# xp3i4/linear

Hardware: AMD Instinct MI355X
Metric: reads/sec (whole node) + HBM GB/s on seed lookup, 10 kb reads vs GRCh38 (higher is better)
Workload: dtype u64

## Files before the change

linear_amd/csrc/lnr_hd.h:

```cpp
#pragma once
#include <stdint.h>
#include <limits.h>
#include "ref_sort.h"

namespace lnr {

typedef uint64_t u64;
typedef int64_t i64;
typedef uint32_t u32;
typedef int32_t i32;
typedef uint16_t u16;
typedef uint8_t u8;

struct UP { u64 first, second; };

static const u64 ANCHOR_ZERO = 1ULL << 20;
static const u64 F_END = 1ULL << 60, F_STRAND = 1ULL << 61, F_RECD = 1ULL << 62, F_MAIN = 1ULL << 63;
static const u64 VALUE_MASK_DSTR = ((1ULL << 60) - 1) | F_STRAND;
static const u64 MAX_CORD_ID = (1ULL << 10) - 1, MAX_CORD_X = (1ULL << 30) - 1;

LNR_HD inline u64 cord_x(u64 v) { return (v >> 20) & ((1ULL << 30) - 1); }
LNR_HD inline u64 cord_y(u64 v) { return v & 0xfffffULL; }
LNR_HD inline u64 cord_strand(u64 v) { return (v >> 61) & 1ULL; }
LNR_HD inline u64 cord_id(u64 v) { return (v >> 50) & 1023ULL; }
LNR_HD inline u64 cord_x40(u64 v) { return (v >> 20) & 0xffffffffffULL; }
LNR_HD inline u64 mk_cord(u64 idx, u64 y, u64 s) { return (idx << 20) + y + (s << 61); }
LNR_HD inline u64 create_cord(u64 id, u64 x, u64 y, u64 s) { return mk_cord((id << 30) + x, y, s); }
LNR_HD inline u64 shift_cord(u64 v, i64 x, i64 y) { return x < 0 ? v - ((u64)(-x) << 20) + (u64)y : v + ((u64)x << 20) + (u64)y; }
LNR_HD inline bool is_end(u64 v) { return (v & F_END) != 0; }
LNR_HD inline u64 hit2cord(u64 a) { return ((a + ((a & 0xfffffULL) << 20) - (ANCHOR_ZERO << 20)) & VALUE_MASK_DSTR) & ~(1ULL << 62); }
LNR_HD inline u64 anchor_x(u64 a) { return cord_x(hit2cord(a)); }
LNR_HD inline i64 labs64(i64 v) { return v < 0 ? -v : v; }
LNR_HD inline i64 max64(i64 a, i64 b) { return a > b ? a : b; }
LNR_HD inline i64 min64(i64 a, i64 b) { return a < b ? a : b; }
LNR_HD inline u64 umin64(u64 a, u64 b) { return a < b ? a : b; }
LNR_HD inline u64 umax64(u64 a, u64 b) { return a > b ? a : b; }
LNR_HD inline int consecutive(u64 c1, u64 c2, u64 thd) {
    u64 x1 = cord_x(c1), x2 = cord_x(c2), y1 = cord_y(c1), y2 = cord_y(c2);
    return !cord_strand(c1 ^ c2) && x1 <= x2 && y1 <= y2 && x2 - x1 < thd && y2 - y1 < thd;
}
LNR_HD inline UP forward_y(UP se, u64 L) {
    UP r;
    if (cord_strand(se.first)) { r.first = L - cord_y(se.second) - 1; r.second = L - cord_y(se.first) - 1; }
    else { r.first = cord_y(se.first); r.second = cord_y(se.second); }
    return r;
}

LNR_HD inline bool lnr_is_leader() {
#if defined(__HIP_DEVICE_COMPILE__)
    return (threadIdx.x & 63) == 0;
#else
    return true;
#endif
}
LNR_HD inline void lnr_wave_sync() {
#if defined(__HIP_DEVICE_COMPILE__)
    __builtin_amdgcn_fence(__ATOMIC_RELEASE, "workgroup");
    __builtin_amdgcn_wave_barrier();
    __builtin_amdgcn_fence(__ATOMIC_ACQUIRE, "workgroup");
#endif
}
LNR_HD inline u32 lnr_uni32(u32 v) {
#if defined(__HIP_DEVICE_COMPILE__)
    return (u32)__builtin_amdgcn_readfirstlane((int)v);
#else
    return v;
#endif
}
LNR_HD inline u64 lnr_uni64(u64 v) { return ((u64)lnr_uni32((u32)(v >> 32)) << 32) | (u64)lnr_uni32((u32)v); }
template <class T>
struct Vec {
    T *p; u32 n, cap; int *ovf;
    LNR_HD void init(T *p_, u32 cap_, int *ovf_) { p = p_; n = 0; cap = cap_; ovf = ovf_; }
    LNR_HD void push(const T &v) { if (n < cap) p[n++] = v; else *ovf = 1; }
    LNR_HD void push_u(const T &v) {
        if (n < cap) { if (lnr_is_leader()) p[n] = v; n++; }
        else if (lnr_is_leader()) *ovf = 1;
    }
    LNR_HD T &operator[](u32 i) { return p[i]; }
    LNR_HD T &back() { return p[n - 1]; }
};
struct Arena {
    char *base; u64 off, cap; int ovf; Arena *next;
    LNR_HD void init(void *b, u64 c) { base = (char *)b; off = 0; cap = c; ovf = 0; next = nullptr; }
    template <class T> LNR_HD T *get(u64 n) {
        u64 bytes = (n * sizeof(T) + 15) & ~15ULL;
        Arena *a = this;
        while (a->off + bytes > a->cap) {
            if (!a->next) { a->ovf = 1; ovf = 1; return (T *)base; }
            a = a->next;
        }
        T *r = (T *)(a->base + a->off);
        a->off += bytes;
        return r;
    }
};
LNR_HD inline u64 job_scratch_bytes(u64 cap) { return (cap + 2) * 160 + 1024; }
LNR_HD inline u64 tail_scratch_bytes(u64 cap) { return cap * 240 + 8192; }

LNR_HD inline int lnr_popc64(u64 v) {
#if defined(__HIP_DEVICE_COMPILE__)
    return __popcll(v);
#else
    return __builtin_popcountll(v);
#endif
}
struct PackedSeq {
    const u64 *pk; const u32 *nm; u64 L;
    LNR_HD u8 operator[](u64 i) const {
        u64 j = i < L ? i : L;
        u32 n = nm[j >> 5]; u64 w = pk[j >> 5];
        u32 v = (u32)(w >> (2 * (j & 31))) & 3;
        return (u8)(((n >> (j & 31)) & 1) ? 4 : v);
    }
    LNR_HD int sum20(u64 p) const {
        u64 w = p >> 5; u32 sh = (u32)(p & 31);
        u64 lo = pk[w], hi = pk[w + 1];
        u64 bits = sh ? (lo >> (2 * sh)) | (hi << (64 - 2 * sh)) : lo;
        bits &= (1ULL << 40) - 1;
        u64 nb = ((((u64)nm[w + 1] << 32) | nm[w]) >> sh) & ((1ULL << 20) - 1);
        return lnr_popc64(bits & 0x5555555555555555ULL) + 2 * lnr_popc64(bits & 0xAAAAAAAAAAAAAAAAULL) + 4 * lnr_popc64(nb);
    }
};
struct ByteSeq {
    const u8 *p; u64 L;
    LNR_HD u8 operator[](u64 i) const { if (i >= L) return 0; u8 b = p[i]; return b > 4 ? (u8)4 : b; }
};
struct SeedOut { u32 X; u32 Y; u32 strand; };

template <int SPAN, class Seq> LNR_HD inline int shape_init_skip_t(const Seq &s) {
    u64 k = 0, count = 0;
    while (count < (u64)SPAN) {
        if (s[k + count] == 4) { k += count + 1; count = 0; }
        else count++;
    }
    return (int)k;
}
template <class Seq> LNR_HD inline int shape_init_skip(const Seq &s) { return shape_init_skip_t<21>(s); }
template <int SPAN, class Seq> LNR_HD inline int shape_const_t(const Seq &s, u64 init_at, int ks, u64 k0) {
    int a = 0, b = 0;
    for (int i = 0; i < SPAN - 1; i++) { a += s[init_at + ks + i]; b += s[k0 + i]; }
    return -3 * SPAN + 2 * a - 2 * b;
}
template <class Seq> LNR_HD inline int shape_const(const Seq &s, u64 init_at, int ks, u64 k0) { return shape_const_t<21>(s, init_at, ks, k0); }
LNR_HD inline int shape_const(const PackedSeq &s, u64 init_at, int ks, u64 k0) {
    return -63 + 2 * s.sum20(init_at + (u64)ks) - 2 * s.sum20(k0);
}
template <int SPAN, int WEIGHT, class Seq> LNR_HD inline SeedOut seed_sample_t(const Seq &s, u64 k, u64 k0, u64 init_at, int ks, int C) {
    u64 h = 0, crh = 0;
    int W = 0;
    u64 n = k - k0 + 1;
    int stale = n < (u64)SPAN ? (int)(SPAN - n) : 0;
    for (int p = 0; p < SPAN; p++) {
        u64 real = s[k + p];
        W += (int)real;
        u64 v = p < stale ? (u64)s[init_at + ks + n - 1 + p] : real;
        h = (h << 2) + v;
        crh |= ((3 - v) & 3) << (2 * p);
    }
    int x = C + 2 * W;
    u64 v2 = x > 0 ? (h & ((1ULL << (2 * SPAN)) - 1)) : crh;
    u64 X = (1ULL << (2 * SPAN)) - 1, t = 0;
    for (unsigned kk = 64 - 2 * SPAN; kk <= 64 - 2 * WEIGHT; kk += 2) {
        u64 v1 = v2 << kk >> (64 - 2 * WEIGHT);
        if (X > v1) { X = v1; t = kk; }
    }
    u64 Y = 0;
    if (x > 0) {
        i64 d = (i64)(t >> 1) + SPAN + WEIGHT - 32;
        for (i64 i = d; i < d + 4; i++) { u64 val = s[(u64)((i64)k + i)]; Y = val > 3 ? (Y << 2) : (Y << 2) + val; }
    } else {
        i64 d = 31 - WEIGHT - (i64)(t >> 1);
        for (i64 i = d; i > d - 4; i--) { i64 val = 3 - (i64)s[(u64)((i64)k + i)]; Y = val < 0 ? (Y << 2) : (Y << 2) + (u64)val; }
    }
    SeedOut o; o.X = (u32)X; o.Y = (u32)Y; o.strand = x > 0 ? 0 : 1;
    return o;
}
template <class Seq> LNR_HD inline SeedOut seed_sample(const Seq &s, u64 k, u64 k0, u64 init_at, int ks, int C) { return seed_sample_t<21, 13>(s, k, k0, init_at, ks, C); }
LNR_HD inline u64 lnr_brev64(u64 v) {
#if defined(__HIP_DEVICE_COMPILE__)
    return __brevll(v);
#else
    v = ((v >> 1) & 0x5555555555555555ULL) | ((v & 0x5555555555555555ULL) << 1);
    v = ((v >> 2) & 0x3333333333333333ULL) | ((v & 0x3333333333333333ULL) << 2);
    v = ((v >> 4) & 0x0F0F0F0F0F0F0F0FULL) | ((v & 0x0F0F0F0F0F0F0F0FULL) << 4);
    v = ((v >> 8) & 0x00FF00FF00FF00FFULL) | ((v & 0x00FF00FF00FF00FFULL) << 8);
    v = ((v >> 16) & 0x0000FFFF0000FFFFULL) | ((v & 0x0000FFFF0000FFFFULL) << 16);
    return (v >> 32) | (v << 32);
#endif
}
LNR_HD inline bool seed_sample_packed(const u64 *pk, const u32 *nm, u64 k, u64 k0, int C, SeedOut &o) {
    if (k - k0 + 1 < 21 || k < 4) return false;
    u64 s0 = k - 4;
    u64 w = s0 >> 5;
    u32 sh = (u32)(s0 & 31);
    u64 nbits = (((u64)nm[w + 1] << 32) | nm[w]) >> sh;
    if (nbits & ((1ULL << 29) - 1)) return false;
    u64 lo = pk[w], hi = pk[w + 1];
    u64 span = sh ? (lo >> (2 * sh)) | (hi << (64 - 2 * sh)) : lo;
    const u64 M42 = (1ULL << 42) - 1;
    u64 win = (span >> 8) & M42;
    int W = lnr_popc64(win & 0x5555555555555555ULL) + 2 * lnr_popc64(win & 0xAAAAAAAAAAAAAAAAULL);
    int x = C + 2 * W;
    u64 v2;
    if (x > 0) {
        u64 r = lnr_brev64(win) >> 22;
        v2 = ((r & 0x2AAAAAAAAAAULL) >> 1) | ((r & 0x15555555555ULL) << 1);
    } else v2 = (~win) & M42;
    u32 v2lo = (u32)v2, v2hi = (u32)(v2 >> 32);
    u32 best = 0xffffffffu;
#pragma unroll
    for (u32 i = 0; i < 9; i++) {
        u32 p = 16 - 2 * i;
        u32 f = p ? ((v2lo >> p) | (v2hi << (32 - p))) : v2lo;
        u32 key = ((f & 0x3ffffffu) << 4) | i;
        best = key < best ? key : best;
    }
    u64 X = best >> 4, t = 22 + 2 * (best & 15u);
    u32 Y;
    if (x > 0) {
        u32 q = (u32)(t >> 1) + 2 + 4;
        u32 b = (u32)(span >> (2 * q)) & 0xFF;
// ... 502 lines not shown
    i32 dx = (i32)((u32)(c11 >> 20) & 0x3fffffffu) - (i32)((u32)(c22 >> 20) & 0x3fffffffu);
    if (dx < 0 || dy < 0 || cord_strand(c11 ^ c22) || dx > 20000 || dy > 20000) return INT_MIN;
    u32 ux = (u32)dx, uy = (u32)dy;
    u32 da = ux > uy ? ux - uy : uy - ux;
    u32 D = uy > 100u ? uy : 100u; D = D > ux ? D : ux;
#if defined(__HIP_DEVICE_COMPILE__)
    float inv = __builtin_amdgcn_rcpf((float)D);
#else
    float inv = 1.0f / (float)D;
#endif
    u32 n = 100u * da;
    u32 q = (u32)((float)n * inv);
    i32 r = (i32)(n - q * D);
    q = r < 0 ? q - 1 : ((u32)r >= D ? q + 1 : q);
    if (da > 100u || q > 50u) {
        if (ux < uy) return (int)(100 - 30) - (int)(uy / 1000u) - (int)(ux / 100u);
        return (int)(100 - 30) - (int)(uy / 100u) - (int)(ux / 1000u);
    }
    return 100 - (int)(uy / 95u);
}
LNR_HD inline int block_score3(u64 c11, u64 c12, u64 c21, u64 c22, u64 L, int strand) {
    i64 dx, dy;
    if (cord_strand(c11) != (u64)strand) {
        if (cord_strand(c22) != (u64)strand) { dy = (i64)(cord_y(c21) - cord_y(c12)); dx = (i64)(cord_x(c21) - cord_x(c12)); }
        else { dy = (i64)(L - cord_y(c12) - 1 - cord_y(c22)); dx = (i64)(cord_x(c11) - cord_x(c22)); }
    } else {
        if (cord_strand(c22) != (u64)strand) { dy = (i64)(cord_y(c11) - L + 1 + cord_y(c21)); dx = (i64)(cord_x(c11) - cord_x(c22)); }
        else { dy = (i64)(cord_y(c11) - cord_y(c22)); dx = (i64)(cord_x(c11) - cord_x(c22)); }
    }
    int f_type = (int)cord_strand(c11 ^ c22);
    i64 thd_min_dx = -(i64)L;
    i64 thd_max_dy = (i64)((float)L * 1.0f);
    i64 dx_ = labs64(dx), dy_ = labs64(dy), da = dx - dy;
    int score = 0;
    if (dy < -80 || dy > thd_max_dy || dx < thd_min_dx || dx_ > 15000) score = INT_MIN;
    else {
        i64 sdy = dy_ > 2000 ? min64(dy_ / 25 - 50, 70) : dy_ / 40;
        i64 sdx = dx_ > 2000 ? min64(dx_ / 25 - 50, 70) : dx_ / 40;
        if (f_type == 1) { if (dx > thd_min_dx) score = (int)(75 - sdy); }
        else if (da < -max64(dx_ / 4, 50)) { if (dx > -50) score = (int)(80 - sdx); else score = (int)(80 - sdy); }
        else if (da > max64(dy / 4, 50)) score = (int)(80 - sdy);
        else score = (int)(100 - sdy);
    }
    return score;
}
LNR_HD inline void best_chains2(const u64 *hits, const UP *sep, const i32 *sep_score, u32 nb, Rec r, u64 L, int which, int strand) {
    for (u32 i = 0; i < nb; i++) {
        int j_str = (int)i - 20 < 0 ? 0 : (int)i - 20;
        int max_j = (int)i, best = -1;
        for (u32 j = (u32)j_str; j < i; j++) {
            int sc = which == 2 ? block_score2(hits[sep[j].first], hits[sep[i].second - 1])
                                : block_score3(hits[sep[j].first], hits[sep[j].second - 1], hits[sep[i].first], hits[sep[i].second - 1], L, strand);
            if (sc > 0 && sc + r.score[j] + sep_score[i] >= best) { max_j = (int)j; best = sc + r.score[j] + sep_score[i]; }
        }
        if (best > 0) {
            r.p2[i] = max_j; r.score[i] = best; r.len[i] = (i32)(sep[i].second - sep[i].first) + r.len[max_j]; r.score2[i] = best;
            r.root[i] = r.root[max_j]; r.leaf[i] = 1; r.leaf[max_j] = 0;
        } else {
            r.p2[i] = -1; r.score[i] = sep_score[i]; r.len[i] = (i32)(sep[i].second - sep[i].first); r.score2[i] = r.score[i];
            r.root[i] = (i32)i; r.leaf[i] = 1;
        }
    }
}
struct BlockScratch { u32 *ptr; UP *sep_tmp; i32 *score_tmp; Rec rec; i32 *chain, *chain_sc, *cnt; LeaderScratch *ls; };
LNR_HD inline void chain_blocks_prepare(const u64 *records, const UP *sep, const i32 *sep_score, u32 nb, int f_sort, BlockScratch s) {
    if (f_sort) {
        u64 *e = (u64 *)s.sep_tmp;
        for (u32 i = 0; i < nb; i++) e[i] = (cord_x40(records[sep[i].first]) << 24) | (u64)i;
        ref_sort(e, (long)nb, [](const u64 &a, const u64 &b) { return (a >> 24) > (b >> 24); }, s.ls->st);
        for (u32 i = 0; i < nb; i++) s.ptr[i] = (u32)(e[i] & 0xffffffu);
    } else {
        for (u32 i = 0; i < nb; i++) s.ptr[i] = i;
    }
    for (u32 i = 0; i < nb; i++) { s.sep_tmp[i] = sep[s.ptr[i]]; s.score_tmp[i] = sep_score[s.ptr[i]]; }
}
LNR_HD inline void chain_blocks_trace(BlockSink &sink, u32 nb, BlockScratch s) {
    sink.elements = s.sep_tmp;
    traceback(s.rec, nb, sink, s.chain, s.chain_sc, s.cnt, 1, 0, 3, 0.7f, *s.ls);
}
LNR_HD inline void chain_blocks_base(BlockSink &sink, const u64 *records, const UP *sep, const i32 *sep_score, u32 nb, u64 L, int which, int strand,
                                     int f_sort, BlockScratch s) {
    if (nb < 2) return;
    chain_blocks_prepare(records, sep, sep_score, nb, f_sort, s);
    best_chains2(records, s.sep_tmp, s.score_tmp, nb, s.rec, L, which, strand);
    chain_blocks_trace(sink, nb, s);
}
LNR_HD inline u32 filter_blocks_hits(const BlockSink &ch, const u64 *hits, u64 *out) {
    if (ch.nchains == 0) return 0xffffffffu;
    u32 n = 0;
    u64 len_current = 0;
    for (i32 i = ch.off[0]; i < ch.off[1]; i++) {
        for (u64 j = ch.el[i].first; j < ch.el[i].second; j++) out[n++] = hits[j] & ~F_END;
        len_current += ch.el[i].second - ch.el[i].first;
    }
    out[n - 1] |= F_END;
    float bound = 0.8 * len_current;
    u32 major_n = 1;
    for (u32 c = 1; c < ch.nchains; c++) {
        len_current = 0;
        for (i32 j = ch.off[c]; j < ch.off[c + 1]; j++) len_current += ch.el[j].second - ch.el[j].first;
        bool f_append = false;
        if (major_n < 5 && (float)len_current > bound) { f_append = true; ++major_n; }
        if (f_append) {
            for (i32 j = ch.off[c]; j < ch.off[c + 1]; j++)
                for (u64 k = ch.el[j].first; k < ch.el[j].second; k++) out[n++] = hits[k] & ~F_END;
            out[n - 1] |= F_END;
        }
        out[n - 1] |= F_END;
    }
    return n;
}

template <bool COOP = true>
LNR_HD inline u32 window_best3(FeatView f1, FeatView f2, u64 y, u64 x0, u64 &x_min) {
#if defined(__HIP_DEVICE_COMPILE__)
    if (!COOP) {
        u32 mn1 = ~0u;
        for (u64 x = x0; x < x0 + 3; x++) { u32 t = wdist_raw(f1, f2, y, x); if (t < mn1) { mn1 = t; x_min = x; } }
        return mn1;
    }
    int lane = (int)(threadIdx.x & 63);
    u32 t = lane < 3 ? wdist_raw(f1, f2, y, x0 + (u64)lane) : 0xffffffffu;
    u32 t0 = __shfl(t, 0), t1 = __shfl(t, 1), t2 = __shfl(t, 2);
    u32 mn = t0; x_min = x0;
    if (t1 < mn) { mn = t1; x_min = x0 + 1; }
    if (t2 < mn) { mn = t2; x_min = x0 + 2; }
    return mn;
#else
    u32 mn = ~0u;
    for (u64 x = x0; x < x0 + 3; x++) { u32 t = wdist_raw(f1, f2, y, x); if (t < mn) { mn = t; x_min = x; } }
    return mn;
#endif
}
LNR_HD inline u64 previous_window(FeatView f1, FeatView f2, u64 cord) {
    u64 gid = cord_id(cord), strand = cord_strand(cord);
    u64 x_suf = cord_x(cord) >> 4, y_suf = cord_y(cord) >> 4, x_min = 0;
    if (y_suf < 5 || x_suf < 6) return 0;
    u64 y = y_suf - 5;
    u32 mn = window_best3(f1, f2, y, x_suf - 6, x_min);
    if (mn > 36) return 0;
    if (x_suf - x_min > 5) return mk_cord((gid << 30) + ((x_suf - 5) << 4), (x_suf - x_min - 5 + y) << 4, strand);
    return mk_cord((gid << 30) + (x_min << 4), y << 4, strand);
}
LNR_HD inline u64 next_window(FeatView f1, FeatView f2, u64 cord) {
    u64 gid = cord_id(cord), strand = cord_strand(cord);
    u64 x_pre = cord_x(cord) >> 4, y_pre = cord_y(cord) >> 4, x_min = 0;
    if (y_pre + 12 > f1.n || x_pre + 12 > f2.n) return 0;
    u64 y = y_pre + 5;
    u32 mn = window_best3(f1, f2, y, x_pre + 3, x_min);
    if (mn > 36) return 0;
    if (x_min - x_pre > 5) return mk_cord((gid << 30) + ((x_pre + 5) << 4), (x_pre + 5 - x_min + y) << 4, strand);
    return mk_cord((gid << 30) + (x_min << 4), y << 4, strand);
}
#if defined(__HIP_DEVICE_COMPILE__)
#if defined(LNR_PROF)
#define PD_CNT(k, v) do { lnr_pd_cnt[k] += (v); } while (0)
#define PD_T0() unsigned long long pd_t0_ = clock64()
#define PD_T(k) do { unsigned long long t_ = clock64(); lnr_pd_cnt[k] += t_ - pd_t0_; pd_t0_ = t_; } while (0)
static __device__ __attribute__((unused)) int lnr_pd_dummy;
#else
#define PD_CNT(k, v) do {} while (0)
#define PD_T0() do {} while (0)
#define PD_T(k) do {} while (0)
#endif
LNR_HD inline bool extend_window(FeatView f1, FeatView f2, Vec<u64> &cords, u64 &tail, u64 cordy_str, u64 cordy_end, unsigned long long *lnr_pd_cnt = nullptr) {
    const int lane = (int)(threadIdx.x & 63);
    (void)lnr_pd_cnt;
    PD_T0();
    u64 *const cp = (u64 *)lnr_uni64((u64)cords.p);
    const u32 ccap = lnr_uni32(cords.cap);
    u32 cn = lnr_uni32(cords.n);
    f1.p = (const F96 *)lnr_uni64((u64)f1.p); f1.n = lnr_uni32(f1.n);
    f2.p = (const F96 *)lnr_uni64((u64)f2.p); f2.n = lnr_uni32(f2.n);
    const u32 p_str = cn - 1;
    tail = lnr_uni64(tail); cordy_str = lnr_uni64(cordy_str); cordy_end = lnr_uni64(cordy_end);
    const int d = lane < 3 ? 1 : (lane < 11 ? 2 : (lane < 26 ? 3 : 4));
    const int pre = d == 1 ? 0 : (d == 2 ? 3 : (d == 3 ? 11 : 26));
    const int la = (lane - pre) / (d + 2), lu = (lane - pre) % (d + 2) - 1;
    int s_ = 1;
    while ((s_ + 1) * (s_ + 1) - 1 <= lane) s_++;
    const int off = lane - (s_ * s_ - 1);
    u32 dvf0;
    {
        u64 x0 = cord_x(tail) >> 4, y0 = cord_y(tail) >> 4;
        dvf0 = lane < 63 ? wdist_raw(f1, f2, y0 + 5 * (u64)s_, x0 + 3 * (u64)s_ + (u64)off) : 0xffffffffu;
    }
    {
        bool stop = false;
        while (!stop) {
            const u64 gid = cord_id(tail), strand = cord_strand(tail);
            const i64 x0 = (i64)(cord_x(tail) >> 4), y0 = (i64)(cord_y(tail) >> 4);
            i64 Y = y0 - 5 * d + la, X = x0 - 5 * d + lu;
            u32 dv = (lane < 50 && Y >= 0 && X >= 0) ? wdist_raw(f1, f2, (u64)Y, (u64)X) : 0xffffffffu;
            PD_CNT(1, 1);
            int a = 0, c = 0;
            for (int k = 0; k < 4; k++) {
                i64 x = x0 - 5 * k + c, y = y0 - 5 * k + a;
                if (y < 5 || x < 6) { stop = true; break; }
                int dd = k + 1;
                int bl = (dd == 1 ? 0 : (dd == 2 ? 3 : (dd == 3 ? 11 : 26))) + a * (dd + 2) + c;
                u32 t0 = (u32)__builtin_amdgcn_readlane((int)dv, bl), t1 = (u32)__builtin_amdgcn_readlane((int)dv, bl + 1), t2 = (u32)__builtin_amdgcn_readlane((int)dv, bl + 2);
                u32 mn = t0; int j = 0;
                if (t1 < mn) { mn = t1; j = 1; }
                if (t2 < mn) { mn = t2; j = 2; }
                if (mn > 36) { stop = true; break; }
                u64 nc;
                if (j == 0) { nc = mk_cord((gid << 30) + ((u64)(x - 5) << 4), (u64)(y - 4) << 4, strand); a++; }
                else { nc = mk_cord((gid << 30) + ((u64)(x - 6 + j) << 4), (u64)(y - 5) << 4, strand); if (j == 2) c++; }
                if (!(cord_y(nc) >= cordy_str)) { stop = true; break; }
                if (cn >= ccap) { if (lnr_is_leader()) *cords.ovf = 1; cords.n = cn; return false; }
                if (lnr_is_leader()) cp[cn] = nc;
                cn++; tail = nc;
            }
        }
    }
    u32 p_end = cn;
    PD_T(6);
    PD_CNT(3, p_end - p_str - 1);
    if (p_end - p_str > 1) {
        PD_CNT(5, 1);
        lnr_wave_sync();
        if (lnr_is_leader())
            for (u32 k = p_str; k < (p_str + p_end) / 2; k++) rs_swap(cp[k], cp[cn - k + p_str - 1]);
        lnr_wave_sync();
        tail = lnr_uni64(cp[cn - 1]);
    }
    PD_T(7);
    {
        bool stop = false, have = true;
        while (!stop) {
            const u64 gid = cord_id(tail), strand = cord_strand(tail);
            const u64 x0 = cord_x(tail) >> 4, y0 = cord_y(tail) >> 4;
            u32 dv = have ? dvf0 : (lane < 63 ? wdist_raw(f1, f2, y0 + 5 * (u64)s_, x0 + 3 * (u64)s_ + (u64)off) : 0xffffffffu);
            have = false;
            PD_CNT(2, 1);
            u64 xc = x0, yc = y0;
            for (int k = 1; k <= 7; k++) {
                if (yc + 12 > f1.n || xc + 12 > f2.n) { stop = true; break; }
                int bl = k * k - 1 + (int)(xc - x0) - 3 * (k - 1);
                u32 t0 = (u32)__builtin_amdgcn_readlane((int)dv, bl), t1 = (u32)__builtin_amdgcn_readlane((int)dv, bl + 1), t2 = (u32)__builtin_amdgcn_readlane((int)dv, bl + 2);
                u32 mn = t0; u64 x_min = xc + 3;
                if (t1 < mn) { mn = t1; x_min = xc + 4; }
                if (t2 < mn) { mn = t2; x_min = xc + 5; }
                if (mn > 36) { stop = true; break; }
                u64 nc = mk_cord((gid << 30) + (x_min << 4), (yc + 5) << 4, strand);
                if (!(cord_y(nc) + 96 < cordy_end)) { stop = true; break; }
                if (cn >= ccap) { if (lnr_is_leader()) *cords.ovf = 1; cords.n = cn; return false; }
                if (lnr_is_leader()) cp[cn] = nc;
                cn++; tail = nc;
                xc = x_min; yc += 5;
                PD_CNT(4, 1);
            }
        }
    }
    PD_T(8);
    cords.n = cn;
    return true;
}
#else
LNR_HD inline bool extend_window(FeatView f1, FeatView f2, Vec<u64> &cords, u64 &tail, u64 cordy_str, u64 cordy_end) {
    u32 p_str = cords.n - 1;
    u64 nc;
    while ((nc = previous_window(f1, f2, tail)) && cord_y(nc) >= cordy_str) {
        if (cords.n >= cords.cap) { *cords.ovf = 1; return false; }
        cords.push(nc); tail = nc;
    }
    u32 p_end = cords.n;
    if (p_end - p_str > 1) {
        for (u32 k = p_str; k < (p_str + p_end) / 2; k++) rs_swap(cords[k], cords[cords.n - k + p_str - 1]);
        tail = cords[cords.n - 1];
    }
    while ((nc = next_window(f1, f2, tail)) && cord_y(nc) + 96 < cordy_end) {
        if (cords.n >= cords.cap) { *cords.ovf = 1; return false; }
        cords.push(nc); tail = nc;
    }
    return true;
}
#endif
struct GenomeFeat { const F96 *base; const u64 *off; u32 nseq; };
LNR_HD inline FeatView f2_view(GenomeFeat g, u64 id) {
    FeatView v;
    if (id >= g.nseq) { v.p = g.base; v.n = 0; return v; }
    v.p = g.base + g.off[id]; v.n = (u32)(g.off[id + 1] - g.off[id]);
    return v;
}
LNR_HD inline void filter_hits_flags(const u64 *hits, u32 nhits, const FeatView f1[2], GenomeFeat g, i32 *keep, u32 first, u32 step) {
    for (u32 it = 1 + first; it < nhits; it += step) {
        u32 dist = wdist_checked(f1[cord_strand(hits[it])], f2_view(g, cord_id(hits[it])), cord_y(hits[it]) >> 4, cord_x(hits[it]) >> 4);
        keep[it] = dist < 50 ? 1 : 0;
    }
}
LNR_HD inline u32 filter_hits_apply(u64 *hits, u32 nhits, const i32 *keep) {
    u32 mv = 0;
    for (u32 it = 1; it < nhits; it++) {
        if (keep[it]) hits[it - mv] = hits[it];
        else mv++;
        if (is_end(hits[it])) hits[it - mv] |= F_END;
    }
    return nhits - mv;
}
LNR_HD inline void path_dst_2(const u64 *hits, u32 nhits, const FeatView f1_[2], GenomeFeat g, Vec<u64> &cords_, u64 read_str, u64 read_end, u64 L) {
    i64 hitBegin = 1, hitEnd = (i64)nhits;
    if (hitBegin >= hitEnd - 1) return;
    Vec<u64> cords = cords_;
    struct NBack { Vec<u64> &dst; Vec<u64> &src; LNR_HD ~NBack() { dst.n = src.n; } } nback_{cords_, cords};
    FeatView f1[2] = {f1_[0], f1_[1]};
    cords.p = (u64 *)lnr_uni64((u64)cords.p); cords.n = lnr_uni32(cords.n); cords.cap = lnr_uni32(cords.cap); cords.ovf = (int *)lnr_uni64((u64)cords.ovf);
    for (int k = 0; k < 2; k++) { f1[k].p = (const F96 *)lnr_uni64((u64)f1[k].p); f1[k].n = lnr_uni32(f1[k].n); }
    g.base = (const F96 *)lnr_uni64((u64)g.base); g.off = (const u64 *)lnr_uni64((u64)g.off); g.nseq = lnr_uni32(g.nseq);
    read_str = lnr_uni64(read_str); read_end = lnr_uni64(read_end); L = lnr_uni64(L);
    hitEnd = (i64)lnr_uni32(nhits);
    u64 tail;
    if (cords.n == 0) { cords.push_u(F_END); tail = F_END; }
    else tail = lnr_uni64(cords[cords.n - 1]);
    u64 ready_str, ready_end, cordy_str = 0, cordy_end = 0;
    bool f_sp_l, f_sp_r = false, f_block_end = false, f_append;
    i64 itt_next = hitBegin + 1, itt_first = hitBegin;
#if defined(LNR_PROF) && defined(__HIP_DEVICE_COMPILE__)
    unsigned long long pdc_[12] = {0, 0, 0, 0, 0, 0, 0, 0, 0, 0, 0, 0}, pdt_ = clock64();
    struct PdPrint { unsigned long long *c; u32 nh; __device__ ~PdPrint() { if ((blockIdx.x % 9973) == 777 && (threadIdx.x & 63) == 0)
        printf("[pd2] block %u: hits %u, visited %llu, extensions %llu, backward frontiers %llu (cords %llu, reversals %llu), forward frontiers %llu (cords %llu); cycles: hit walk %llu, backward %llu, reversal %llu, forward %llu\n",
               blockIdx.x, nh, c[10], c[0], c[1], c[3], c[5], c[2], c[4], c[9], c[6], c[7], c[8]); } } pdp_{pdc_, nhits};
#endif
#if defined(__HIP_DEVICE_COMPILE__)
    const u32 ln_ = threadIdx.x & 63;
    const u64 hreg0 = ln_ < nhits ? hits[ln_] : 0, hreg1 = ln_ + 64 < nhits ? hits[ln_ + 64] : 0;
    auto HIT = [&](i64 i) -> u64 {
        if (i < 128) {
            const u64 r = i < 64 ? hreg0 : hreg1;
            const int l_ = (int)(i & 63);
            return ((u64)(u32)__builtin_amdgcn_readlane((int)(u32)(r >> 32), l_) << 32) | (u64)(u32)__builtin_amdgcn_readlane((int)(u32)r, l_);
        }
        return lnr_uni64(hits[i]);
    };
#else
    auto HIT = [&](i64 i) -> u64 { return hits[i]; };
#endif
    u64 view_id = ~0ULL; FeatView view_f2; view_f2.p = g.base; view_f2.n = 0;
    for (i64 itt = hitBegin; itt < hitEnd; itt = itt_next++) {
        const u64 hi = HIT(itt), hpv = HIT(itt - 1);
        bool first_i = is_end(hpv);
        ready_str = cord_strand(hi) ? L - read_end : read_str;
        ready_end = cord_strand(hi) ? L - read_str + 1 : read_end;
        i64 da_l = first_i ? 0 : labs64((i64)(cord_x(hi) - cord_x(hpv) - cord_y(hi) + cord_y(hpv)));
        f_sp_l = (da_l > 80) || cord_strand(hi ^ hpv);
        while (1) {
            if (itt_next >= hitEnd) { f_block_end = true; itt_first = itt_next; break; }
            const u64 hn = HIT(itt_next), hp = HIT(itt_next - 1);
            if (is_end(hp)) { f_block_end = true; itt_first = itt_next; break; }
            i64 da_r = labs64((i64)(cord_x(hn) - cord_x(hp) - cord_y(hn) + cord_y(hp)));
            f_sp_r = (da_r > 80) || cord_strand(hn ^ hp);
            if ((cord_y(hi) + 96 < cord_y(hn) && cord_x(hi) + 96 < cord_x(hn)) || f_sp_r) break;
            itt_next++;
        }
        f_append = false;
        if (!f_sp_r && !f_block_end) {
            cordy_str = f_sp_l ? hi : (first_i ? ready_str : cord_y(tail));
            cordy_end = cord_y(HIT(itt_next));
            if (cords.n >= cords.cap) { if (lnr_is_leader()) *cords.ovf = 1; return; }
            cords.push_u(hi & ~F_END); tail = hi & ~F_END;
            f_append = true;
        } else {
            const u64 hl = HIT(itt_next - 1);
            if (!f_sp_l && cord_y(hl) >= 96 && cord_x(hl) >= 96) {
                u64 nc = shift_cord(hl, -96, -96);
                cordy_str = first_i ? read_str : cord_y(nc);
                cordy_end = cord_y(hl);
                if (cords.n >= cords.cap) { if (lnr_is_leader()) *cords.ovf = 1; return; }
                cords.push_u(nc & ~F_END); tail = nc & ~F_END;
                f_append = true;
            }
        }
        if (is_end(hi) || f_block_end) { f_block_end = true; cordy_end = ready_end; }
        if (f_append && cord_id(hi) != view_id) { view_id = cord_id(hi); view_f2 = f2_view(g, view_id); }
#if defined(LNR_PROF) && defined(__HIP_DEVICE_COMPILE__)
        { unsigned long long t_ = clock64(); pdc_[9] += t_ - pdt_; pdt_ = t_; pdc_[0] += f_append ? 1 : 0; pdc_[10]++; }
        if (f_append && !extend_window(f1[cord_strand(hi)], view_f2, cords, tail, cordy_str, cordy_end, pdc_)) return;
        pdt_ = clock64();
        if (0)
#endif
        if (f_append && !extend_window(f1[cord_strand(hi)], view_f2, cords, tail, cordy_str, cordy_end)) return;
        if (f_block_end) { tail |= F_END; if (lnr_is_leader()) cords[cords.n - 1] = tail; }
        itt_next = f_block_end ? itt_first : itt_next;
        f_sp_r = false; f_block_end = false;
    }
}

LNR_HD inline u32 clean_blocks(u64 *cords, u32 n, u64 drop_len) {
    if (n == 0) return 0;
    u64 ptr = 1, len = 0;
    for (u32 i = 1; i < n; i++) {
        len++;
        if (!is_end(cords[i - 1])) {
            i64 dx = (i64)(cord_x(cords[i]) - cord_x(cords[ptr - 1]));
            i64 dy = (i64)(cord_y(cords[i]) - cord_y(cords[ptr - 1]));
            if ((dx < 0 || dy < 0) && labs64(dx) < 50 && labs64(dy) < 50) { --len; --ptr; }
            else cords[ptr] = cords[i];
        } else cords[ptr] = cords[i];
        if (is_end(cords[i])) {
            ptr = len < drop_len ? ptr - len : ptr;
            len = 0;
            cords[ptr] |= F_END;
        }
        ptr++;
    }
    return (u32)ptr;
}
LNR_HD inline int gather_gaps_y(UP *str_ends, u32 ns, Vec<UP> &gaps, u64 L, u64 gap_size, LeaderScratch &ls) {
    u64 cord_frt = 0, cord_end = L - 1;
    int sum = 0;
    UP u;
    if (ns == 0) { u.first = cord_frt; u.second = cord_end; gaps.push(u); sum += (int)(cord_y(cord_end) - cord_y(cord_frt)); return sum; }
    ref_sort(str_ends, (long)ns, [L](const UP &i, const UP &j) {
        u64 y1 = cord_strand(i.first) ? L - cord_y(i.second) - 1 : cord_y(i.first);
        u64 y2 = cord_strand(j.first) ? L - cord_y(j.second) - 1 : cord_y(j.first);
        return y1 < y2;
    }, ls.st);
    u64 f_cover = 0, cordy1 = 0, cordy2 = 0;
    UP y1 = forward_y(str_ends[0], L), y2 = y1;
    if (y1.first > gap_size) {
        cordy2 = cord_y(y1.first);
        u.first = cord_frt; u.second = cordy2; gaps.push(u);
        sum += (int)(cord_y(u.second) - cord_y(u.first));
    }
    for (u32 i = 1; i < ns; i++) {
        if (!f_cover) { y1 = forward_y(str_ends[i - 1], L); cordy1 = cord_y(y1.second); }
        y2 = forward_y(str_ends[i], L);
        cordy2 = cord_y(y2.first);
        if (y1.second > y2.second) f_cover = 1;
        else {
            if (y2.first > y1.second && y2.first - y1.second > gap_size) {
                u.first = cordy1; u.second = cordy2; gaps.push(u);
                sum += (int)(cord_y(u.second) - cord_y(u.first));
            }
            f_cover = 0;
        }
    }
    u64 max_y_end = f_cover ? y1.second : y2.second;
    if (L - max_y_end > gap_size) {
        u.first = max_y_end; u.second = cord_end; gaps.push(u);
        sum += (int)(cord_y(u.second) - cord_y(u.first));
    }
    return sum;
}

LNR_HD inline void chain_blocks_single_strand(const u64 *cords, UP *sep, u32 nb, i32 *sep_score, BlockSink &sink, int strand, u64 L, BlockScratch s) {
    if (strand)
        ref_sort(sep, (long)nb, [cords, L](const UP &a, const UP &b) {
            u64 y1 = !cord_strand(cords[a.first]) ? L - 1 - cord_y(cords[a.second - 1]) : cord_y(cords[a.first]);
            u64 y2 = !cord_strand(cords[b.first]) ? L - 1 - cord_y(cords[b.second - 1]) : cord_y(cords[b.first]);
            return y1 > y2;
        }, s.ls->st);
    else
        ref_sort(sep, (long)nb, [cords, L](const UP &a, const UP &b) {
            u64 y1 = cord_strand(cords[a.first]) ? L - 1 - cord_y(cords[a.second - 1]) : cord_y(cords[a.first]);
            u64 y2 = cord_strand(cords[b.first]) ? L - 1 - cord_y(cords[b.second - 1]) : cord_y(cords[b.first]);
            return y1 > y2;
        }, s.ls->st);
    for (u32 i = 0; i < nb; i++) sep_score[i] = (i32)((sep[i].second - sep[i].first) * 16);
    chain_blocks_base(sink, cords, sep, sep_score, nb, L, 3, strand, 0, s);
}
LNR_HD inline int best_strand(const BlockSink &c1, const BlockSink &c2) {
    u32 n = c1.nchains < c2.nchains ? c1.nchains : c2.nchains;
    int l1 = 0, l2 = 0;
    for (u32 i = 0; i < n; i++) {
        for (i32 j = c1.off[i]; j < c1.off[i + 1]; j++) l1 += (int)(c1.el[j].second - c1.el[j].first);
        for (i32 j = c2.off[i]; j < c2.off[i + 1]; j++) l2 += (int)(c2.el[j].second - c2.el[j].first);
        if (l1 < l2) return 1;
        else if (l1 > l2) return 0;
    }
    return 0;
}
LNR_HD inline void revert_chain_block_strand(BlockSink &cc, const u64 *cords, int strand) {
    u64 f_strand = strand ? 1 : 0;
    for (u32 c = 0; c < cc.nchains; c++) {
        UP *el = cc.el + cc.off[c];
        u32 len = (u32)(cc.off[c + 1] - cc.off[c]) + 1;
        u64 swap_str = 0, pre = 0, cur = 0;
        for (u32 j = 0; j < len; j++) {
            if (j == len - 1 || cord_strand(cords[el[j].first]) == f_strand) cur = 0;
            else cur = 1;
            if (cur && !pre) swap_str = j;
            if (!cur && pre)
                for (u32 k = (u32)swap_str; k < (swap_str + j) / 2; k++) rs_swap(el[k], el[swap_str + j - 1 - k]);
            pre = cur;
        }
    }
}
LNR_HD inline u32 filter_blocks_cords(const BlockSink &ch, const u64 *hits, u64 *out, u64 major_limit) {
    if (ch.nchains == 0) return 0xffffffffu;
    u32 n = 0;
    u64 len_current = 0;
    out[n++] = hits[0];
    for (i32 i = ch.off[0]; i < ch.off[1]; i++) {
        for (u64 j = ch.el[i].first; j < ch.el[i].second; j++) out[n++] = hits[j] & ~F_END;
        len_current += ch.el[i].second - ch.el[i].first;
    }
    out[n - 1] |= F_END;
    float bound = 0.8 * len_current;
    u32 major_n = 1;
    for (u32 c = 1; c < ch.nchains && major_n < major_limit; c++) {
        len_current = 0;
        for (i32 j = ch.off[c]; j < ch.off[c + 1]; j++) len_current += ch.el[j].second - ch.el[j].first;
        if ((float)len_current > bound) {
            ++major_n;
            for (i32 j = ch.off[c]; j < ch.off[c + 1]; j++)
                for (u64 k = ch.el[j].first; k < ch.el[j].second; k++) out[n++] = hits[k] & ~F_END;
            out[n - 1] |= F_END;
        }
    }
    return n;
}

struct JobCtx {
    u64 L, read_str, read_end;
    int mode;
    FeatView f1[2];
    GenomeFeat g;
    u16 *bins; u32 nbins;
    u64 *pair_evals;
    unsigned long long *prof;
    int traceback_done;
};
struct JobScratch {
    Vec<u64> hits; Vec<i32> hscore; Vec<UP> sep, tmp;
    Rec rec;
    i32 *chain, *chain_sc, *cnt, *sep_score;
    u32 *xs, *ys;
    u64 *cuts, *xy_strs, *alt;
};
LNR_HD inline bool job_carve(Arena &ar, u32 cap, JobScratch &S, int *ovf) {
    u32 c2 = cap + 2;
// ... 142 lines not shown
```

Measured before the change: 2.613 million.

## Keep backward-walk cords in lane registers and plan hit grouping with wave ballots

The backward window walk now holds its new cords in a per-lane register (one cord per lane, up to 64). It writes them to memory already reversed via a lane shuffle, which replaces the leader-serial in-memory reversal loop and its two wave barriers. Path planning in path_dst_2 precomputes stop and split masks for up to 128 hits with wave ballots. The serial scan for the next far hit becomes a ballot plus find-first-set. This adds complexity, plus a spill fallback when a walk exceeds 64 cords and a host emulation path.

```diff
diff --git a/linear_amd/csrc/lnr_hd.h b/linear_amd/csrc/lnr_hd.h
--- a/linear_amd/csrc/lnr_hd.h
+++ b/linear_amd/csrc/lnr_hd.h
@@ -68,6 +68,27 @@
 #endif
 }
 LNR_HD inline u64 lnr_uni64(u64 v) { return ((u64)lnr_uni32((u32)(v >> 32)) << 32) | (u64)lnr_uni32((u32)v); }
+#if defined(__HIP_DEVICE_COMPILE__)
+#define LNR_FOR_LANES(l, nl) for (u32 l = threadIdx.x & 63, lnr_once_ = 1; lnr_once_; lnr_once_ = 0)
+template <int NL> struct LaneU64 {
+    u64 v;
+    LNR_HD void set(u32 l, u64 x) { if ((threadIdx.x & 63) == l) v = x; }
+    LNR_HD u64 get(u32) const { return v; }
+    LNR_HD u64 from(u32, u32 src) const { return (u64)__shfl((unsigned long long)v, (int)src); }
+};
+template <class F> LNR_HD inline u64 lnr_ballot(u32, F pred) { return (u64)__ballot(pred(threadIdx.x & 63) ? 1 : 0); }
+LNR_HD inline u32 lnr_ctz64(u64 v) { return (u32)__ffsll((unsigned long long)v) - 1; }
+#else
+#define LNR_FOR_LANES(l, nl) for (u32 l = 0; l < (u32)(nl); l++)
+template <int NL> struct LaneU64 {
+    u64 v[NL];
+    LNR_HD void set(u32 l, u64 x) { v[l] = x; }
+    LNR_HD u64 get(u32 l) const { return v[l]; }
+    LNR_HD u64 from(u32, u32 src) const { return v[src]; }
+};
+template <class F> LNR_HD inline u64 lnr_ballot(u32 nl, F pred) { u64 m = 0; for (u32 l = 0; l < nl; l++) if (pred(l)) m |= 1ULL << l; return m; }
+LNR_HD inline u32 lnr_ctz64(u64 v) { return (u32)__builtin_ctzll(v); }
+#endif
 template <class T>
 struct Vec {
     T *p; u32 n, cap; int *ovf;
@@ -876,6 +897,31 @@
     if (x_min - x_pre > 5) return mk_cord((gid << 30) + ((x_pre + 5) << 4), (x_pre + 5 - x_min + y) << 4, strand);
     return mk_cord((gid << 30) + (x_min << 4), y << 4, strand);
 }
+template <int NL> struct ExtBack {
+    LaneU64<NL> reg; bool spilled;
+    LNR_HD void init() { spilled = false; LNR_FOR_LANES(l, NL) reg.set(l, 0); }
+    LNR_HD void store_walk(u64 *cp, u32 p_str, u32 nb) { LNR_FOR_LANES(l, NL) if (l < nb) cp[p_str + 1 + l] = reg.get(l); }
+    LNR_HD void push(u64 *cp, u32 p_str, u32 k, u64 nc) {
+        if (k < (u32)NL) { reg.set(k, nc); return; }
+        if (k == (u32)NL) { store_walk(cp, p_str, (u32)NL); spilled = true; }
+        if (lnr_is_leader()) cp[p_str + 1 + k] = nc;
+    }
+    LNR_HD void overflow(u64 *cp, u32 p_str, u32 nb) { if (!spilled) store_walk(cp, p_str, nb); }
+    LNR_HD void finish(u64 *cp, u32 p_str, u32 nb, u64 entry) {
+        if (nb == 0) return;
+        if (spilled) {
+            lnr_wave_sync();
+            if (lnr_is_leader())
+                for (u32 k = p_str; k < (p_str + p_str + nb + 1) / 2; k++) rs_swap(cp[k], cp[p_str + nb - (k - p_str)]);
+            return;
+        }
+        LNR_FOR_LANES(l, NL) {
+            const u64 s = reg.from(l, l < nb ? nb - 1 - l : 0);
+            if (l < nb) cp[p_str + l] = s;
+        }
+        if (lnr_is_leader()) cp[p_str + nb] = entry;
+    }
+};
 #if defined(__HIP_DEVICE_COMPILE__)
 #if defined(LNR_PROF)
 #define PD_CNT(k, v) do { lnr_pd_cnt[k] += (v); } while (0)
@@ -904,6 +950,8 @@
     int s_ = 1;
     while ((s_ + 1) * (s_ + 1) - 1 <= lane) s_++;
     const int off = lane - (s_ * s_ - 1);
+    const u64 entry = tail;
+    ExtBack<64> bb; bb.init();
     u32 dvf0;
     {
         u64 x0 = cord_x(tail) >> 4, y0 = cord_y(tail) >> 4;
@@ -932,8 +980,8 @@
                 if (j == 0) { nc = mk_cord((gid << 30) + ((u64)(x - 5) << 4), (u64)(y - 4) << 4, strand); a++; }
                 else { nc = mk_cord((gid << 30) + ((u64)(x - 6 + j) << 4), (u64)(y - 5) << 4, strand); if (j == 2) c++; }
                 if (!(cord_y(nc) >= cordy_str)) { stop = true; break; }
-                if (cn >= ccap) { if (lnr_is_leader()) *cords.ovf = 1; cords.n = cn; return false; }
-                if (lnr_is_leader()) cp[cn] = nc;
+                if (cn >= ccap) { bb.overflow(cp, p_str, cn - p_str - 1); if (lnr_is_leader()) *cords.ovf = 1; cords.n = cn; return false; }
+                bb.push(cp, p_str, cn - p_str - 1, nc);
                 cn++; tail = nc;
             }
         }
@@ -943,11 +991,8 @@
     PD_CNT(3, p_end - p_str - 1);
     if (p_end - p_str > 1) {
         PD_CNT(5, 1);
-        lnr_wave_sync();
-        if (lnr_is_leader())
-            for (u32 k = p_str; k < (p_str + p_end) / 2; k++) rs_swap(cp[k], cp[cn - k + p_str - 1]);
-        lnr_wave_sync();
-        tail = lnr_uni64(cp[cn - 1]);
+        bb.finish(cp, p_str, p_end - p_str - 1, entry);
+        tail = entry;
     }
     PD_T(7);
     {
@@ -1000,6 +1045,27 @@
     }
     return true;
 }
+template <int NL>
+LNR_HD inline bool extend_window_lanes(FeatView f1, FeatView f2, Vec<u64> &cords, u64 &tail, u64 cordy_str, u64 cordy_end) {
+    u64 *const cp = cords.p;
+    const u32 p_str = cords.n - 1;
+    const u64 entry = tail;
+    u32 cn = cords.n;
+    u64 nc;
+    ExtBack<NL> bb; bb.init();
+    while ((nc = previous_window(f1, f2, tail)) && cord_y(nc) >= cordy_str) {
+        if (cn >= cords.cap) { bb.overflow(cp, p_str, cn - p_str - 1); *cords.ovf = 1; cords.n = cn; return false; }
+        bb.push(cp, p_str, cn - p_str - 1, nc);
+        cn++; tail = nc;
+    }
+    if (cn - p_str > 1) { bb.finish(cp, p_str, cn - p_str - 1, entry); tail = entry; }
+    cords.n = cn;
+    while ((nc = next_window(f1, f2, tail)) && cord_y(nc) + 96 < cordy_end) {
+        if (cords.n >= cords.cap) { *cords.ovf = 1; return false; }
+        cords.push(nc); tail = nc;
+    }
+    return true;
+}
 #endif
 struct GenomeFeat { const F96 *base; const u64 *off; u32 nseq; };
 LNR_HD inline FeatView f2_view(GenomeFeat g, u64 id) {
@@ -1023,6 +1089,23 @@
     }
     return nhits - mv;
 }
+LNR_HD inline u32 plan_hit_flags(u64 h, u64 hp) {
+    const bool e = is_end(hp);
+    const i64 da = labs64((i64)(cord_x(h) - cord_x(hp) - cord_y(h) + cord_y(hp)));
+    return (u32)(((!e && da > 80) || cord_strand(h ^ hp)) ? 1 : 0) | (u32)(e ? 2 : 0);
+}
+LNR_HD inline bool plan_far(u64 hi, u64 hn) { return cord_y(hi) + 96 < cord_y(hn) && cord_x(hi) + 96 < cord_x(hn); }
+LNR_HD inline u32 plan_first_above(u64 m0, u64 m1, u32 i, u32 n, u32 nl) {
+    if (i + 1 < nl) { const u64 w = m0 & (~0ULL << (i + 1)); if (w) { const u32 j = lnr_ctz64(w); return j < n ? j : n; } }
+    if (i + 1 < 2 * nl) { const u64 w = m1 & (~0ULL << (i + 1 > nl ? i + 1 - nl : 0)); if (w) { const u32 j = nl + lnr_ctz64(w); return j < n ? j : n; } }
+    return n;
+}
+#if defined(__HIP_DEVICE_COMPILE__)
+#define LNR_PLAN_NL 64
+#else
+#define LNR_PLAN_NL 0
+#endif
+template <int NL = LNR_PLAN_NL>
 LNR_HD inline void path_dst_2(const u64 *hits, u32 nhits, const FeatView f1_[2], GenomeFeat g, Vec<u64> &cords_, u64 read_str, u64 read_end, u64 L) {
     i64 hitBegin = 1, hitEnd = (i64)nhits;
     if (hitBegin >= hitEnd - 1) return;
@@ -1057,9 +1140,24 @@
         }
         return lnr_uni64(hits[i]);
     };
+    auto HLANE = [&](u32 r, u32) -> u64 { return r ? hreg1 : hreg0; };
 #else
     auto HIT = [&](i64 i) -> u64 { return hits[i]; };
-#endif
+    auto HLANE = [&](u32 r, u32 l) -> u64 { return (i64)(l + r * NL) < hitEnd ? hits[l + r * NL] : 0; };
+#endif
+    const bool planned = NL > 0 && hitEnd <= 2 * (i64)NL;
+    constexpr u32 NLD = NL > 0 ? (u32)NL : 1u;
+    u64 p_stop0 = 0, p_stop1 = 0, p_split0 = 0, p_split1 = 0;
+    const bool two = planned && hitEnd > (i64)NL;
+    if (planned) {
+        auto fl = [&](u32 j) -> u32 { return j >= 1 && (i64)j < hitEnd ? plan_hit_flags(hits[j], hits[j - 1]) : 0u; };
+        p_stop0 = lnr_ballot((u32)NL, [&](u32 l) { return fl(l) != 0; });
+        p_split0 = lnr_ballot((u32)NL, [&](u32 l) { return (fl(l) & 1) != 0; });
+        if (two) {
+            p_stop1 = lnr_ballot((u32)NL, [&](u32 l) { return fl(l + NL) != 0; });
+            p_split1 = lnr_ballot((u32)NL, [&](u32 l) { return (fl(l + NL) & 1) != 0; });
+        }
+    }
     u64 view_id = ~0ULL; FeatView view_f2; view_f2.p = g.base; view_f2.n = 0;
     for (i64 itt = hitBegin; itt < hitEnd; itt = itt_next++) {
         const u64 hi = HIT(itt), hpv = HIT(itt - 1);
@@ -1068,6 +1166,14 @@
         ready_end = cord_strand(hi) ? L - read_str + 1 : read_end;
         i64 da_l = first_i ? 0 : labs64((i64)(cord_x(hi) - cord_x(hpv) - cord_y(hi) + cord_y(hpv)));
         f_sp_l = (da_l > 80) || cord_strand(hi ^ hpv);
+        if (planned) {
+            const u64 m0 = p_stop0 | lnr_ballot((u32)NL, [&](u32 l) { return (i64)l < hitEnd && plan_far(hi, HLANE(0, l)); });
+            const u64 m1 = !two ? 0 : p_stop1 | lnr_ballot((u32)NL, [&](u32 l) { return (i64)(l + NL) < hitEnd && plan_far(hi, HLANE(1, l)); });
+            const u32 j = plan_first_above(m0, m1, (u32)itt, (u32)hitEnd, (u32)NL);
+            itt_next = (i64)j;
+            if (itt_next >= hitEnd || is_end(HIT(itt_next - 1))) { f_block_end = true; itt_first = itt_next; }
+            else f_sp_r = (((j < NLD ? p_split0 : p_split1) >> (j % NLD)) & 1) != 0;
+        } else
         while (1) {
             if (itt_next >= hitEnd) { f_block_end = true; itt_first = itt_next; break; }
             const u64 hn = HIT(itt_next), hp = HIT(itt_next - 1);
@@ -1102,6 +1208,10 @@
         if (f_append && !extend_window(f1[cord_strand(hi)], view_f2, cords, tail, cordy_str, cordy_end, pdc_)) return;
         pdt_ = clock64();
         if (0)
+#endif
+#if !defined(__HIP_DEVICE_COMPILE__)
+        if (NL > 0) { if (f_append && !extend_window_lanes<(int)NLD>(f1[cord_strand(hi)], view_f2, cords, tail, cordy_str, cordy_end)) return; }
+        else
 #endif
         if (f_append && !extend_window(f1[cord_strand(hi)], view_f2, cords, tail, cordy_str, cordy_end)) return;
         if (f_block_end) { tail |= F_END; if (lnr_is_leader()) cords[cords.n - 1] = tail; }
```

New measurement: 2.611 million. No clear change (-0.1%).
